# pansanity666/TransHuman

Hardware: AMD Instinct MI355X
Metric: rays/sec (512x512, 64 samples/ray) (higher is better)
Workload: dtype f32 (fp16 hi/lo x3 MFMA emulation)

## Files before the change

### transhuman_amd/csrc/k_mlp_fused8_kernel.h

```cpp
#pragma once
#include "k_mlp_fused_kernel.h"

typedef float f8_f4 __attribute__((ext_vector_type(4)));
typedef short f8_s4 __attribute__((ext_vector_type(4)));
typedef short f8_s8 __attribute__((ext_vector_type(8)));

#define F8_THREADS 512
#define F8_PART_FLOATS (3 * 8 * 32)
#define F8_PSTR 12
#define F8_MISC_FLOATS (F8_PSTR * 32 + F8_PART_FLOATS + 32 + 8)
#define F8_LDS_BYTES (ABUF_BYTES + MBUF_BYTES + F8_MISC_FLOATS * 4)
static_assert(F8_LDS_BYTES <= 163840, "the 8-wave tile must fit the CU's LDS");

#define F8_MFMA(A, B, C) __builtin_amdgcn_mfma_f32_16x16x32_f16((A), (B), (C), 0, 0, 0)

template <int CT>
__device__ __forceinline__ void f8_load_w(const uint4* __restrict__ wl, int t, uint4 (&w)[CT][2]) {
    const uint4* p = wl + (long long)t * (CT * 2 * 64);
#pragma unroll
    for (int c = 0; c < CT; ++c) {
        w[c][0] = p[(c * 2 + 0) * 64];
        w[c][1] = p[(c * 2 + 1) * 64];
    }
}
// ... 115 lines not shown
__device__ __forceinline__ void f8_gemm_rt(const char* __restrict__ ahi, const char* __restrict__ alo, int str,
                                           const uint4* __restrict__ wp, int T, int lane, f8_f4 (&acc)[CT][RT], uint4 (&w)[2][CT][2]) {
    if constexpr (RT % 3 == 0) f8_gemm3<RT, CT, ROWSTEP, PERM, PRE>(ahi, alo, str, wp, T, lane, acc, w);
    else f8_gemm<RT, CT, ROWSTEP, PERM, PRE>(ahi, alo, str, wp, T, lane, acc, w);
}

template <int STR, bool NONNEG = true>
__device__ __forceinline__ void f8_store_h(const f8_f4& t, int row, int col0, char* __restrict__ hi, char* __restrict__ lo, int lane,
                                           unsigned& rm) {
    const int c = col0 + 4 * (lane >> 4);
    uint2 a, b;
    split_pair(t[0], t[1], a.x, b.x);
    split_pair(t[2], t[3], a.y, b.y);
    range_acc<NONNEG>(rm, a.x);
    range_acc<NONNEG>(rm, a.y);
    *reinterpret_cast<uint2*>(hi + row * STR + 2 * c) = a;
    *reinterpret_cast<uint2*>(lo + row * STR + 2 * c) = b;
}
__device__ __forceinline__ f8_f4 f8_finish(const f8_f4& a, const float4& b, float inv_scale, bool relu) {
    const f32x2 sc = {inv_scale, inv_scale};
    f32x2 y01 = __builtin_elementwise_fma((f32x2){a[0], a[1]}, sc, (f32x2){b.x, b.y});
    f32x2 y23 = __builtin_elementwise_fma((f32x2){a[2], a[3]}, sc, (f32x2){b.z, b.w});
    if (relu) {
        y01 = __builtin_elementwise_max(y01, (f32x2){0.f, 0.f});
        y23 = __builtin_elementwise_max(y23, (f32x2){0.f, 0.f});
    }
    return (f8_f4){y01[0], y01[1], y23[0], y23[1]};
}
__device__ __forceinline__ float f8_xor(float v, int lane, int mask) {
    return __builtin_bit_cast(float, __builtin_amdgcn_ds_bpermute((lane ^ mask) << 2, __builtin_bit_cast(int, v)));
}
__device__ __forceinline__ float4 f8_bias(const float* __restrict__ bias, int col0, int lane) {
    return *reinterpret_cast<const float4*>(bias + col0 + 4 * (lane >> 4));
}

template <int RT, int NV, int H, int R0, bool FIRST>
__device__ __forceinline__ void f8_mfma_dual(const uint4 (&r3)[2][2], const uint4 (&ra)[1][2], const h8 (&mh)[1], const h8 (&ml)[1],
                                             const h8 (&xh)[NV], const h8 (&xl)[NV], f8_f4 (&a3)[2][2], f8_f4 (&va)[1][RT]) {
    const f8_f4 zero = {0.f, 0.f, 0.f, 0.f};
#pragma unroll
    for (int t = 0; t < 3; ++t) {
        const int wp = t == 0 ? 1 : 0;
        const bool lo = t == 1;
        const bool first = FIRST && t == 0;
        a3[0][H] = F8_MFMA(*reinterpret_cast<const h8*>(&r3[0][wp]), lo ? ml[0] : mh[0], first ? zero : a3[0][H]);
#pragma unroll
        for (int r = 0; r < NV; ++r) {
            va[0][R0 + r] = F8_MFMA(*reinterpret_cast<const h8*>(&ra[0][wp]), lo ? xl[r] : xh[r], first ? zero : va[0][R0 + r]);
            if (r == 0) a3[1][H] = F8_MFMA(*reinterpret_cast<const h8*>(&r3[1][wp]), lo ? ml[0] : mh[0], first ? zero : a3[1][H]);
        }
    }
}

template <int V>
__global__ __launch_bounds__(F8_THREADS, 2) void mlp_fused8_kernel(FusedParams P_arg) {
#define PK P_arg
    struct F8Dbg { long long* dbg; };
    const F8Dbg P{PK.dbg};
    extern __shared__ __attribute__((aligned(16))) char lds[];
    char* abuf = lds;
    char* mbuf = lds + ABUF_BYTES;
    float* misc = reinterpret_cast<float*>(lds + ABUF_BYTES + MBUF_BYTES);
    float* probs = misc;
    float* part = misc + F8_PSTR * 32;
    float* sig = part + F8_PART_FLOATS;
    int* flag = reinterpret_cast<int*>(sig + 32);

    const int tid = threadIdx.x, lane = tid & 63, wave = tid >> 6;
    const int l15 = lane & 15, g4 = lane >> 4;
    const int tile = (int)((blockIdx.x & 7) * (gridDim.x >> 3) + (blockIdx.x >> 3));
    const int pbase = tile * FM_PTS;
    if (pbase >= PK.P) return;
    const int npts = min(FM_PTS, PK.P - pbase);
    const int fm_dbg_tile = tile;
    const int zoff = 0;
    constexpr int ROWS = 32 * V, RT = 2 * V;
    constexpr int RS256 = 16 * STR256;
    int dbg_i = 1;
    long long dbg_t = 0;
    long long* dbg_keep = reinterpret_cast<long long*>(flag + 2);
    constexpr float inv_v = 1.0f / (float)V;
    unsigned rmax = 0u;
    unsigned seen_s = 0u, seen_p = 0u, seen_n = 0u, seen_i = 0u, seen_4 = 0u;
    char* a256_lo = abuf + ROWS * STR256;

    struct TexPre { unsigned h0, h1; fm_u4 rq; };
    auto tex_fetch = [&]() __attribute__((always_inline)) {
        int tl = tile;
        asm volatile("" : "+s"(tl));
        TexPre t;
        const unsigned* hb = PK.tex_hdr + (long long)tl * 512;
        t.h0 = hb[lane];
        t.h1 = hb[64 + lane];
        t.rq = (fm_u4){0u, 0u, 0u, 0u};
        if (tid < 64 * V) t.rq = *reinterpret_cast<const fm_u4*>(PK.tex_rec + (long long)tl * V * 32 * 8 + tid * 4);
        return t;
    };
    auto fill_tex = [&](const TexPre& pre, auto rgb, auto&& under) __attribute__((always_inline)) {
        constexpr bool RGB = decltype(rgb)::value;
        constexpr int TSTR = 1040, TMAX = 103, NK = (TMAX + 7) / 8, NR = 4 * V;
        static_assert(TMAX * TSTR <= ABUF_BYTES, "a pass of texel rows must fit the operand buffer");
        int wv = __builtin_amdgcn_readfirstlane(wave), tl = tile;
        asm volatile("" : "+s"(wv), "+s"(tl));
        const unsigned* hb = PK.tex_hdr + (long long)tl * 512;
        unsigned h0 = pre.h0, h1 = pre.h1;
        const int npass = __builtin_amdgcn_readfirstlane((int)(h0 >> 16));
        char* recl = reinterpret_cast<char*>(misc);
        static_assert(32 * V * 32 <= (F8_PSTR * 32 + F8_PART_FLOATS) * 4, "row records must fit probs + part");
        unsigned fv[NR][4] = {};
        f32x2 bias_lo = {0.f, 0.f}, bias_hi = {0.f, 0.f};
        if constexpr (!RGB) {
            const float4 b4 = *reinterpret_cast<const float4*>(PK.ar0.bias + 4 * lane);
            bias_lo = (f32x2){b4.x, b4.y};
            bias_hi = (f32x2){b4.z, b4.w};
        }
        for (int p = 0; p < npass; ++p) {
            if (p > 0) {
                FM_SYNCL();
                h0 = hb[p * 128 + lane];
                h1 = hb[p * 128 + 64 + lane];
            }
            const int U = __builtin_amdgcn_readfirstlane((int)(h0 & 0xffffu));
            {
                constexpr int NA = 7, NB = 10;
                const char* mbase = reinterpret_cast<const char*>(RGB ? PK.tex_map2 : PK.tex_map);
                const unsigned loff = (unsigned)lane * 16u;
                const int last = U - 1;
                fm_u4 ta[NA], tb[NB - NA], tc[NK - NB];
#pragma unroll
                for (int k = 0; k < NA; ++k) {
                    const int i = min(wv + 8 * k, last);
                    const unsigned id = (unsigned)__builtin_amdgcn_readlane((int)h0, 8 + i);
                    ta[k] = *reinterpret_cast<const fm_u4*>(mbase + TX_ADDR(id));
                }
                const bool more = U > 8 * NA, most = U > 8 * NB;
                if (more) {
#pragma unroll
                    for (int k = NA; k < NB; ++k) {
                        const int i = min(wv + 8 * k, last);
                        const unsigned id = (unsigned)__builtin_amdgcn_readlane((int)h1, i - 56);
                        tb[k - NA] = *reinterpret_cast<const fm_u4*>(mbase + TX_ADDR(id));
                    }
                }
                if (most) {
#pragma unroll
                    for (int k = NB; k < NK; ++k) {
                        const int i = min(wv + 8 * k, last);
                        const unsigned id = (unsigned)__builtin_amdgcn_readlane((int)h1, i - 56);
                        tc[k - NB] = *reinterpret_cast<const fm_u4*>(mbase + TX_ADDR(id));
                    }
                }
                if (p == 0) {
                    under();
                    if (tid < 64 * V) *reinterpret_cast<fm_u4*>(recl + tid * 16) = pre.rq;
                }
                int wv2 = wv;
                asm volatile("" : "+s"(wv2));
#pragma unroll
                for (int k = 0; k < NA; ++k) *reinterpret_cast<fm_u4*>(abuf + min(wv2 + 8 * k, last) * TSTR + lane * 16) = ta[k];
                if (more) {
#pragma unroll
                    for (int k = NA; k < NB; ++k) *reinterpret_cast<fm_u4*>(abuf + min(wv2 + 8 * k, last) * TSTR + lane * 16) = tb[k - NA];
                }
                if (most) {
#pragma unroll
                    for (int k = NB; k < NK; ++k) *reinterpret_cast<fm_u4*>(abuf + min(wv2 + 8 * k, last) * TSTR + lane * 16) = tc[k - NB];
                }
            }
            FM_SYNCL();
            const int sh2 = npass == 1 ? 2 : npass == 2 ? 1 : 0;
            const int cofs = lane * 16;
            struct RowIn { float4 a, b, c, d; fm_u4 q0; };
            auto issue = [&](int k, const fm_u4& o, RowIn& r) __attribute__((always_inline)) {
                r.q0 = *reinterpret_cast<const fm_u4*>(recl + (wv + 8 * k) * 32);
                r.a = *reinterpret_cast<const float4*>(abuf + (o[0] + cofs));
                r.b = *reinterpret_cast<const float4*>(abuf + (o[1] + cofs));
                r.c = *reinterpret_cast<const float4*>(abuf + (o[2] + cofs));
                r.d = *reinterpret_cast<const float4*>(abuf + (o[3] + cofs));
            };
            auto offs = [&](int k) __attribute__((always_inline)) {
                return *reinterpret_cast<const fm_u4*>(recl + (wv + 8 * k) * 32 + 16);
            };
            auto blend = [&](int k, const RowIn& r, auto sel) __attribute__((always_inline)) {
                const unsigned u0 = r.q0[0], u1 = r.q0[1], u2 = r.q0[2], u3 = r.q0[3];
                const float w00 = __builtin_bit_cast(float, u0), w01 = __builtin_bit_cast(float, u1),
                            w10 = __builtin_bit_cast(float, u2), w11 = __builtin_bit_cast(float, u3);
                const f32x2 W00 = {w00, w00}, W01 = {w01, w01}, W10 = {w10, w10}, W11 = {w11, w11};
                f32x2 lo = (f32x2){r.a.x, r.a.y} * W00, hi = (f32x2){r.a.z, r.a.w} * W00;
                lo = __builtin_elementwise_fma((f32x2){r.b.x, r.b.y}, W01, lo);
                hi = __builtin_elementwise_fma((f32x2){r.b.z, r.b.w}, W01, hi);
                lo = __builtin_elementwise_fma((f32x2){r.c.x, r.c.y}, W10, lo);
                hi = __builtin_elementwise_fma((f32x2){r.c.z, r.c.w}, W10, hi);
                lo = __builtin_elementwise_fma((f32x2){r.d.x, r.d.y}, W11, lo);
                hi = __builtin_elementwise_fma((f32x2){r.d.z, r.d.w}, W11, hi);
                unsigned n0, n1, n2, n3;
                if constexpr (RGB) {
                    const float l0 = lo[0], l1 = lo[1], h0f = hi[0], h1f = hi[1];
                    n0 = __builtin_bit_cast(unsigned, l0); n1 = __builtin_bit_cast(unsigned, l1);
                    n2 = __builtin_bit_cast(unsigned, h0f); n3 = __builtin_bit_cast(unsigned, h1f);
                } else {
                    lo = __builtin_elementwise_max(lo + bias_lo, (f32x2){0.f, 0.f});
                    hi = __builtin_elementwise_max(hi + bias_hi, (f32x2){0.f, 0.f});
                    split_pair(lo[0], lo[1], n0, n2);
                    split_pair(hi[0], hi[1], n1, n3);
                }
                if constexpr (decltype(sel)::value) {
                    const bool mine = ((k & 3) >> sh2) == p;
                    fv[k][0] = mine ? n0 : fv[k][0]; fv[k][1] = mine ? n1 : fv[k][1];
                    fv[k][2] = mine ? n2 : fv[k][2]; fv[k][3] = mine ? n3 : fv[k][3];
                } else {
                    fv[k][0] = n0; fv[k][1] = n1; fv[k][2] = n2; fv[k][3] = n3;
                }
            };
            auto rows_loop = [&](auto sel) __attribute__((always_inline)) {
                RowIn in[2];
                fm_u4 of[2];
                of[0] = offs(0);
                of[1] = offs(1);
                issue(0, of[0], in[0]);
#pragma unroll
                for (int k = 0; k < NR; ++k) {
                    if (k + 1 < NR) issue(k + 1, of[(k + 1) & 1], in[(k + 1) & 1]);
                    if (k + 2 < NR) of[k & 1] = offs(k + 2);
                    FM_SB();
                    blend(k, in[k & 1], sel);
                    FM_SB();
                }
            };
            if (npass == 1) rows_loop(std::false_type{});
            else rows_loop(std::true_type{});
        }
        FM_SYNCL();
        if constexpr (RGB) {
#pragma unroll
            for (int k = 0; k < NR; ++k)
                *reinterpret_cast<fm_u4*>(abuf + (wv + 8 * k) * TSTR + lane * 16) = (fm_u4){fv[k][0], fv[k][1], fv[k][2], fv[k][3]};
        } else {
#pragma unroll
            for (int k = 0; k < NR; ++k) {
                range_acc<true>(rmax, fv[k][0]);
                range_acc<true>(rmax, fv[k][1]);
                *reinterpret_cast<uint2*>(abuf + (wv + 8 * k) * STR256 + lane * 8) = make_uint2(fv[k][0], fv[k][1]);
                *reinterpret_cast<uint2*>(a256_lo + (wv + 8 * k) * STR256 + lane * 8) = make_uint2(fv[k][2], fv[k][3]);
            }
            range_commit(PK.range, TH_RANGE_P, seen_p, rmax);
        }
    };

    if (PK.dbg != nullptr && tid == 0 && (tile & 15) == 0) {
        atomicAdd(reinterpret_cast<unsigned long long*>(PK.dbg), 1ull);
        dbg_t = clock64();
        dbg_keep[0] = dbg_t;
        dbg_keep[1] = wall_clock64();
    }
    fm_u4 rv4 = {0u, 0u, 0u, 0u};
    unsigned rv1 = 0u;
    static_assert(TH_RANGE_S == 1 && TH_RANGE_P == 2 && TH_RANGE_N == 3 && TH_RANGE_INTER == 4 && TH_RANGE_F4 == 5, "range slots 1..5");
    if (PK.range != nullptr) {
        const unsigned* rtab = PK.range + zoff;
        rv4 = (fm_u4){rtab[1], rtab[2], rtab[3], rtab[4]};
        rv1 = rtab[5];
    }
    TexPre tex_pre = tex_fetch(), tex_pre2;

    int vsel[2] = {0, 0};
    float vdv[2] = {0.f, 0.f};
    f8_f4 acc2[2][RT];
    {
        constexpr int STOK_STR = 1040;
        static_assert(32 * V * STOK_STR <= ABUF_BYTES, "T' rows must fit the operand buffer");
        char* pe_hi = mbuf;
        char* pe_lo = mbuf + 32 * STR64;
        const int pt = tid & 255, prow = pt >> 3, pc = pt & 7, ppl = tid >> 8;
        const int psrc = min(prow, npts - 1);
        const uint4 pe_v = *reinterpret_cast<const uint4*>(PK.pe + (long long)(pbase + psrc) * 128 + 64 * ppl + 8 * pc);
        char* wsp_hi = mbuf + 16384;
        char* wsp_lo = wsp_hi + 32 * STRVD;
        const unsigned* hdr = reinterpret_cast<const unsigned*>(PK.stok) + (long long)((PK.P + 31) / 32 * 32) * 16 + (long long)tile * 128;
        const unsigned h0 = hdr[lane], h1 = hdr[64 + lane];
        const int ns = tid / 7, nk = tid - 7 * ns;
        int slot = -1;
        float nw = 0.f;
        if (tid < 224) {
// ... 240 lines not shown
                    f8_store_h<STR256>(n, (2 * i + h) * 16 + l15, wave * 32 + c * 16, abuf, a256_lo, lane, rmax);
                }
            }
        }
        range_commit(PK.range, TH_RANGE_N, seen_n, rmax);
    }

    uint4 wk2[2][2][2];
    FM_SB();
    f8_load_w<2>(F8_WSLICE(PK.w16.fc_2, wave, 2) + lane, 0, wk2[0]);
#pragma unroll
    for (int q = 0; q < 2; ++q) {
        const int i = tid + F8_THREADS * q, row = i >> 5, c = i & 31;
        int x = pbase + row;
        if (PK.vd_sel != nullptr && PK.rgb_all != 2 && c < 27 && row < npts) x = PK.vd_sel[pbase + row];
        vsel[q] = x;
    }
    FM_SYNCL();
    f8_gemm_rt<RT, 2, RS256, true, true>(abuf, a256_lo, STR256, F8_WSLICE(PK.w16.fc_2, wave, 2), 8, lane, acc2, wk2);
    const float4 bi[2] = {f8_bias(PK.fc_2.bias, wave * 32, lane), f8_bias(PK.fc_2.bias, wave * 32 + 16, lane)};
#pragma unroll
    for (int q = 0; q < 2; ++q) {
        const int i = tid + F8_THREADS * q, row = i >> 5, c = i & 31;
        float x = 0.f;
        if (PK.rgb_all != 2 && c < 27 && row < npts) {
            const long long vr = PK.vd_sel ? (long long)(vsel[q] / PK.vd_div) : (long long)(pbase + row);
            x = PK.vd[vr * 27 + c];
        }
        vdv[q] = x;
    }
    FM_SYNCL();
#pragma unroll
    for (int c = 0; c < 2; ++c) {
#pragma unroll
        for (int r = 0; r < RT; ++r) acc2[c][r] = f8_finish(acc2[c][r], bi[c], PK.fc_2.inv_scale, true);
#pragma unroll
        for (int h = 0; h < 2; ++h) {
            f8_f4 m = acc2[c][h];
#pragma unroll
            for (int r = 1; r < V; ++r) m = m + acc2[c][2 * r + h];
            m = m * (f8_f4){inv_v, inv_v, inv_v, inv_v};
            f8_store_h<STR256>(m, h * 16 + l15, wave * 32 + c * 16, mbuf, mbuf + 32 * STR256, lane, rmax);
        }
#pragma unroll
        for (int r = 0; r < RT; ++r) f8_store_h<STR256>(acc2[c][r], r * 16 + l15, wave * 32 + c * 16, abuf, a256_lo, lane, rmax);
    }
    range_commit(PK.range, TH_RANGE_INTER, seen_i, rmax);
    FM_SYNCL();

    char* vd_hi = mbuf + MBUF_VD_OFF;
    char* vd_lo = vd_hi + 32 * STRVD;
    tex_pre2 = tex_fetch();
    f8_f4 va[1][RT];
    {
        f8_f4 a3[2][2];
        const float4 aw[2] = {f8_bias(PK.alpha_w, wave * 32, lane), f8_bias(PK.alpha_w, wave * 32 + 16, lane)};
        const float4 b3[2] = {f8_bias(PK.fc_3.bias, wave * 32, lane), f8_bias(PK.fc_3.bias, wave * 32 + 16, lane)};
        if (PK.rgb_all != 2) {
            constexpr int T = 8;
            const uint4* w3l = F8_WSLICE(PK.w16.fc_3, wave, 2) + lane;
            const uint4* wal = F8_WSLICE(PK.w16.vfA, wave, 1) + lane;
            const int aoff = f8_aoff<true>(lane, STR256);
            const char* mhi = mbuf;
            const char* mlo = mbuf + 32 * STR256;
            uint4 r3[2][2][2], ra[2][1][2];
            h8 mah[1], mal[1], xah[V], xal[V], mbh[1], mbl[1], xbh[V], xbl[V];
            f8_load_w<2>(w3l, 0, r3[0]);
            f8_load_w<1>(wal, 0, ra[0]);
            f8_load_x<1, RS256, true>(mhi, mlo, aoff, 0, mah, mal);
            f8_load_x<V, RS256, true>(abuf, a256_lo, aoff, 0, xah, xal);
            FM_SB();
            auto step = [&](auto first, auto par, int t) __attribute__((always_inline)) {
                constexpr bool F = decltype(first)::value;
                constexpr int PB = decltype(par)::value;
                const int tn = t + 1 < T ? t + 1 : T - 1;
                f8_load_x<1, RS256, true>(mhi + RS256, mlo + RS256, aoff, t, mbh, mbl);
                f8_load_x<V, RS256, true>(abuf + V * RS256, a256_lo + V * RS256, aoff, t, xbh, xbl);
                f8_load_w<2>(w3l, tn, r3[PB ^ 1]);
                f8_load_w<1>(wal, tn, ra[PB ^ 1]);
                f8_mfma_dual<RT, V, 0, 0, F>(r3[PB], ra[PB], mah, mal, xah, xal, a3, va);
                f8_interleave<2 + 2 * V + 6, 3 * (2 + V)>();
                f8_load_x<1, RS256, true>(mhi, mlo, aoff, tn, mah, mal);
                f8_load_x<V, RS256, true>(abuf, a256_lo, aoff, tn, xah, xal);
                f8_mfma_dual<RT, V, 1, V, F>(r3[PB], ra[PB], mbh, mbl, xbh, xbl, a3, va);
                f8_interleave<2 + 2 * V, 3 * (2 + V)>();
            };
            step(std::true_type{}, std::integral_constant<int, 0>{}, 0);
            step(std::false_type{}, std::integral_constant<int, 1>{}, 1);
#pragma unroll 1
            for (int t = 2; t < T; t += 2) {
                step(std::false_type{}, std::integral_constant<int, 0>{}, t);
                step(std::false_type{}, std::integral_constant<int, 1>{}, t + 1);
            }
        } else {
#pragma unroll
            for (int r = 0; r < RT; ++r) va[0][r] = (f8_f4){0.f, 0.f, 0.f, 0.f};
            uint4 w3[2][2][2];
            f8_gemm<2, 2, RS256, true, false>(mbuf, mbuf + 32 * STR256, STR256, F8_WSLICE(PK.w16.fc_3, wave, 2), 8, lane, a3, w3);
        }
        float s2[2];
#pragma unroll
        for (int h = 0; h < 2; ++h) {
            float s = 0.f;
#pragma unroll
            for (int c = 0; c < 2; ++c) {
                const f8_f4 y = f8_finish(a3[c][h], b3[c], PK.fc_3.inv_scale, true);
                s = fmaf(y[0], aw[c].x, s);
                s = fmaf(y[1], aw[c].y, s);
                s = fmaf(y[2], aw[c].z, s);
                s = fmaf(y[3], aw[c].w, s);
            }
            s += f8_xor(s, lane, 16);
            s += f8_xor(s, lane, 32);
            s2[h] = s;
        }
        if (g4 == 0) part[wave * 32 + l15] = s2[0];
        if (g4 == 1) part[wave * 32 + 16 + l15] = s2[1];
        if (tid == 0) *flag = 0;
        FM_SYNCL();
        if (tid < 32) {
            float sg = PK.alpha_b[zoff];
#pragma unroll
            for (int w = 0; w < 8; ++w) sg += part[w * 32 + tid];
            sig[tid] = sg;
            if (tid < npts && PK.rgb_all != 2 && (PK.rgb_all == 1 || sg > 0.f)) *flag = 1;
        }
#pragma unroll
        for (int q = 0; q < 2; ++q) {
            const int i = tid + F8_THREADS * q, row = i >> 5, c = i & 31;
            _Float16 a, b;
            split_h(vdv[q], a, b);
            *reinterpret_cast<_Float16*>(vd_hi + row * STRVD + 2 * c) = a;
            *reinterpret_cast<_Float16*>(vd_lo + row * STRVD + 2 * c) = b;
        }
        FM_SYNCL();
    }
    const bool need_rgb = *flag != 0;
    float rgb_out[3] = {0.f, 0.f, 0.f};
    if (need_rgb) {
        uint4 wvd[1][2];
        f8_load_w<1>(F8_WSLICE(PK.w16.vfD, wave, 1) + lane, 0, wvd);
        FM_SB();
        fill_tex(tex_pre2, std::true_type{}, [&]() __attribute__((always_inline)) {
            h8 xh[2], xl[2];
            f8_load_x<2, 16 * STRVD, false>(vd_hi, vd_lo, f8_aoff<false>(lane, STRVD), 0, xh, xl);
#pragma unroll
            for (int r = 0; r < RT; ++r) {
                va[0][r] = F8_MFMA(*reinterpret_cast<const h8*>(&wvd[0][1]), xh[r & 1], va[0][r]);
                va[0][r] = F8_MFMA(*reinterpret_cast<const h8*>(&wvd[0][0]), xl[r & 1], va[0][r]);
                va[0][r] = F8_MFMA(*reinterpret_cast<const h8*>(&wvd[0][0]), xh[r & 1], va[0][r]);
            }
        });
        FM_SYNCL();
        uint4 w4[4][1][2];
        {
            const uint4* wl4 = F8_WSLICE(PK.w16.fc_4, wave, 1) + lane;
#pragma unroll
            for (int t = 0; t < 4; ++t) f8_load_w<1>(wl4, t, w4[t]);
        }
        float4 rw[3];
#pragma unroll
        for (int o = 0; o < 3; ++o) rw[o] = f8_bias(PK.rgb_w + o * 128, wave * 16, lane);
        const float4 b4 = f8_bias(PK.fc_4.bias, wave * 16, lane);
        const float4 bt = f8_bias(PK.rst.bias, wave * 16, lane), br = f8_bias(PK.rst.bias, 128 + wave * 16, lane);
        char* f4_hi = mbuf + MBUF_FC4_OFF;
        char* f4_lo = f4_hi + 32 * STR128;
        {
            const char* mb = abuf + l15 * 1040 + 4 * (wave * 16 + 4 * g4);
            f8_f4 u[RT];
#pragma unroll
            for (int r = 0; r < RT; ++r) {
                const float4 m1 = *reinterpret_cast<const float4*>(mb + r * 16 * 1040);
                const float4 m2 = *reinterpret_cast<const float4*>(mb + r * 16 * 1040 + 512);
                const f8_f4 t = f8_finish(va[0][r], bt, PK.rst.inv_scale, false);
                const f32x2 z2 = {0.f, 0.f};
                const f32x2 u01 = __builtin_elementwise_max((f32x2){t[0], t[1]} + (f32x2){m1.x, m1.y}, z2) + ((f32x2){m2.x, m2.y} + (f32x2){br.x, br.y});
                const f32x2 u23 = __builtin_elementwise_max((f32x2){t[2], t[3]} + (f32x2){m1.z, m1.w}, z2) + ((f32x2){m2.z, m2.w} + (f32x2){br.z, br.w});
                u[r] = (f8_f4){u01[0], u01[1], u23[0], u23[1]};
            }
#pragma unroll
            for (int h = 0; h < 2; ++h) {
                f8_f4 m = u[h];
#pragma unroll
                for (int r = 1; r < V; ++r) m = m + u[2 * r + h];
                m = m * (f8_f4){inv_v, inv_v, inv_v, inv_v};
                f8_store_h<STR128, false>(m, h * 16 + l15, wave * 16, f4_hi, f4_lo, lane, rmax);
            }
            range_commit(PK.range, TH_RANGE_F4, seen_4, rmax);
        }
        FM_SYNCL();
        f8_f4 a4[1][2];
        {
            const int aoff4 = f8_aoff<false>(lane, STR128);
#pragma unroll
// ... 48 lines not shown
```

### transhuman_amd/csrc/k_mlp_fused_host.hip

```cpp
#include <stdio.h>
#include <stdlib.h>
#include <string.h>

#include "k_mlp_fused_kernel.h"
#include "k_mlp_fused8_kernel.h"

__global__ void pack_fused_kernel(const float* __restrict__ W, int N, int K, int KB, int CT, const int* __restrict__ cols,
                                  float scale, uint4* __restrict__ out) {
    long long total = 4LL * KB * CT * 2 * 64;
    for (long long o = blockIdx.x * (long long)blockDim.x + threadIdx.x; o < total;
         o += (long long)gridDim.x * blockDim.x) {
        int lane = (int)(o & 63);
        long long q = o >> 6;
        int plane = (int)(q & 1); q >>= 1;
        int ct = (int)(q % CT); q /= CT;
        int kb = (int)(q % KB);
        int wave = (int)(q / KB);
        int col = cols[wave * CT + ct] + (lane & 31);
        int k0 = 16 * kb + 8 * (lane >> 5);
        h8 v;
#pragma unroll
        for (int j = 0; j < 8; ++j) {
            int k = k0 + j;
            float x = (col < N && k < K) ? W[(long long)col * K + k] * scale : 0.f;
// ... 310 lines not shown
    hipLaunchKernelGGL(absmax_kernel, dim3(64), dim3(256), 0, s, tprime, (long long)rows * 256, amax);
    hipLaunchKernelGGL(tok_split_kernel, dim3(th_cdiv(rows, 4) < 1024 ? th_cdiv(rows, 4) : 1024), dim3(256), 0, s, tprime, rows, sc,
                       range);
    TH_LAUNCH_CHECK();
    return 0;
}

int th_map_fold_launch(const FusedParams& base, const float* map_split, int V, int H, int W, const int32_t* box, float* fold,
                       unsigned int* range, hipStream_t s, const unsigned* demand) {
    TH_REQUIRE(base.compact_ready, "the map fold needs the colour-folded layers (th_mlp_weights.upsample_color)");
    TH_REQUIRE(V >= 1 && H >= 1 && W >= 1 && map_split && fold, "bad argument");
    MapFoldParams p;
    p.ar0 = base.ar0c; p.rst = base.rstc;
    p.lat = map_split; p.rgb = map_split + (size_t)V * H * W * 256;
    p.box = box; p.V = V; p.H = H; p.W = W;
    p.out0 = fold; p.out12 = fold + (size_t)V * H * W * 256;
    p.range = range;
    p.list = nullptr; p.count = nullptr;
    static unsigned long long attr_done = 0ull;
    if (th_lds_attr_needed(&attr_done)) {
        TH_HIP(hipFuncSetAttribute((const void*)map_fold_kernel<false>, hipFuncAttributeMaxDynamicSharedMemorySize, 2 * MF_TEX * STR272));
        TH_HIP(hipFuncSetAttribute((const void*)map_fold_kernel<true>, hipFuncAttributeMaxDynamicSharedMemorySize, 2 * MF_TEX * STR272));
    }
    if (demand != nullptr) {
        const size_t NW = (size_t)V * H * W / 32;
        p.count = demand + 2 * NW;
        p.list = reinterpret_cast<const int32_t*>(demand + 2 * NW + 16);
        hipLaunchKernelGGL(map_fold_kernel<true>, dim3(512), dim3(256), 2 * MF_TEX * STR272, s, p);
        TH_LAUNCH_CHECK();
        return 0;
    }
    const int tpr = (W + MF_TEX - 1) / MF_TEX;
    hipLaunchKernelGGL(map_fold_kernel<false>, dim3((unsigned)(V * H * tpr)), dim3(256), 2 * MF_TEX * STR272, s, p);
    TH_LAUNCH_CHECK();
    return 0;
}

int th_mlp_fused_forward(const FusedParams& base, const ThMlpPacked& heads, int V, int P, const float* stok,
                         const void* pe, const void* f, int f_ld, const float* vd, const int32_t* vd_sel, int vd_div, int rgb_all, float* raw_c,
                         unsigned int* range, hipStream_t s, const void* tsplit, const float* t_inv, int t_nc, const float* tex_map,
                         size_t tex_stride) {
    if (P <= 0) return 0;
    TH_REQUIRE(V >= 1 && V <= 3, "fused MLP supports 1..3 reference views");
    TH_REQUIRE(f_ld == 384 || (f_ld == 272 && base.compact_ready),
               "pixel-feature rows must be 384 wide, or 272 wide with upsample_color weights uploaded");
    const bool cf = f_ld == 272;
    FusedParams p = base;
    if (cf) { p.ar0 = base.ar0c; p.rst = base.rstc; }
    p.alpha_w = heads.alpha_w; p.alpha_b = heads.alpha_b; p.rgb_w = heads.rgb_w; p.rgb_b = heads.rgb_b;
    TH_REQUIRE(tsplit == nullptr || (t_inv != nullptr && t_nc >= 7 && t_nc <= 4096), "split token table: scale word and 7 <= N_c <= 4096");
    p.tsplit = (const _Float16*)tsplit; p.t_inv = t_inv; p.t_nc = t_nc;
    const bool tex = tex_map != nullptr;
    TH_REQUIRE(!tex || (cf && f != nullptr), "texel hand-over: compact (272-wide) operand planes only");
    p.tex_hdr = nullptr; p.tex_rec = nullptr; p.tex_map = nullptr; p.tex_map2 = nullptr;
    if (tex) {
        p.tex_hdr = (const unsigned*)f;
        p.tex_rec = p.tex_hdr + (size_t)th_cdiv(P, FM_PTS) * 512;
        p.tex_map = tex_map;
        p.tex_map2 = tex_map + tex_stride;
        f = nullptr;
    }
    p.stok = stok; p.pe = (const _Float16*)pe; p.f = (const _Float16*)f; p.vd = vd; p.vd_sel = vd_sel; p.vd_div = vd_div > 0 ? vd_div : 1; p.raw_c = raw_c; p.P = P; p.rgb_all = rgb_all; p.range = range;
    static unsigned long long attr_done = 0ull;
    if (th_lds_attr_needed(&attr_done)) {
#define FM_ATTR(V_, F_)                                                                                       \
    TH_HIP(hipFuncSetAttribute((const void*)mlp_fused_kernel<V_, F_>, hipFuncAttributeMaxDynamicSharedMemorySize, \
                               FUSED_LDS_BYTES))
        FM_ATTR(1, 0); FM_ATTR(2, 0); FM_ATTR(3, 0); FM_ATTR(1, 1); FM_ATTR(2, 1); FM_ATTR(3, 1);
#undef FM_ATTR
#define FM_ATTR_T(V_)                                                                                              \
    TH_HIP(hipFuncSetAttribute((const void*)mlp_fused_kernel<V_, 1, true>, hipFuncAttributeMaxDynamicSharedMemorySize, \
                               FUSED_LDS_BYTES))
        FM_ATTR_T(1); FM_ATTR_T(2); FM_ATTR_T(3);
#undef FM_ATTR_T
    }
    dim3 grid(tex ? 8 * th_cdiv(th_cdiv(P, FM_PTS), 8) : th_cdiv(P, FM_PTS));
    const bool eight = base.waves == 8 && tex && tsplit != nullptr;
    static unsigned long long attr8_done = 0ull;
    if (eight && th_lds_attr_needed(&attr8_done)) {
        TH_HIP(hipFuncSetAttribute((const void*)mlp_fused8_kernel<1>, hipFuncAttributeMaxDynamicSharedMemorySize, F8_LDS_BYTES));
        TH_HIP(hipFuncSetAttribute((const void*)mlp_fused8_kernel<2>, hipFuncAttributeMaxDynamicSharedMemorySize, F8_LDS_BYTES));
        TH_HIP(hipFuncSetAttribute((const void*)mlp_fused8_kernel<3>, hipFuncAttributeMaxDynamicSharedMemorySize, F8_LDS_BYTES));
    }
    static int dbg_state = getenv("TH_FUSED_DBG") ? 1 : 0;
    static long long* dbg_dev = nullptr;
    p.dbg = base.cycles_buf;
    const bool dbg_now = dbg_state == 1 && P >= 4096 && base.cycles_buf == nullptr;
    hipEvent_t dbg_e0 = nullptr, dbg_e1 = nullptr;
    if (dbg_now) {
        if (!dbg_dev) TH_HIP(hipMalloc((void**)&dbg_dev, 64 * sizeof(long long)));
        TH_HIP(hipMemsetAsync(dbg_dev, 0, 64 * sizeof(long long), s));
        p.dbg = dbg_dev;
        TH_HIP(hipEventCreate(&dbg_e0));
        TH_HIP(hipEventCreate(&dbg_e1));
        TH_HIP(hipStreamSynchronize(s));
        TH_HIP(hipEventRecord(dbg_e0, s));
    }
#define FM_LAUNCH(V_, F_) hipLaunchKernelGGL((mlp_fused_kernel<V_, F_>), grid, dim3(256), FUSED_LDS_BYTES, s, p)
#define FM_LAUNCH_T(V_) hipLaunchKernelGGL((mlp_fused_kernel<V_, 1, true>), grid, dim3(256), FUSED_LDS_BYTES, s, p)
#define FM_LAUNCH_8(V_) hipLaunchKernelGGL((mlp_fused8_kernel<V_>), grid, dim3(F8_THREADS), F8_LDS_BYTES, s, p)
    if (eight) {
        if (V == 1) FM_LAUNCH_8(1); else if (V == 2) FM_LAUNCH_8(2); else FM_LAUNCH_8(3);
    } else if (tex) {
        if (V == 1) FM_LAUNCH_T(1); else if (V == 2) FM_LAUNCH_T(2); else FM_LAUNCH_T(3);
    } else
    switch (V * 2 + (cf ? 1 : 0)) {
        case 2: FM_LAUNCH(1, 0); break;
        case 3: FM_LAUNCH(1, 1); break;
// ... 33 lines not shown
```

### transhuman_amd/csrc/th_internal.h

```cpp
#pragma once
#include <hip/hip_runtime.h>
#include <stdint.h>
#include <stddef.h>
#include <time.h>
#include <string>

#include "transhuman_hip.h"

#define TH_WAVE 64

void th_set_error(const std::string& msg);
#define TH_FAIL(msg)                                                                \
    do {                                                                            \
        th_set_error(std::string(__func__) + ": " + (msg));                         \
        return -1;                                                                  \
    } while (0)
#define TH_REQUIRE(cond, msg)                                                       \
    do {                                                                            \
        if (!(cond)) TH_FAIL(msg);                                                  \
    } while (0)
#define TH_HIP(call)                                                                \
    do {                                                                            \
        hipError_t e__ = (call);                                                    \
        if (e__ != hipSuccess) {                                                    \
// ... 157 lines not shown
}

#endif

struct ThMlpPacked {
    ThPacked fc_0, alpha_res_0, kv0, kv1, fc_1, fc_2, fc_3, feature_fc, rgb_res_0, view_fc, rgb_res_1, fc_4;
    ThPacked fc_0tok;
    ThPacked alpha_res_0c, rgb_res_0c, rgb_res_1c;
    bool compact_ready = false;
    float *alpha_w = nullptr, *alpha_b = nullptr;
    float *rgb_w = nullptr, *rgb_b = nullptr;
    bool ready = false;
};
struct ThVitBlockPacked {
    float *ln1_w, *ln1_b, *ln2_w, *ln2_b;
    ThPacked qkv, proj, fc1, fc2;
};
struct ThVitPacked {
    int depth = 0, dim = 0, heads = 0;
    ThVitBlockPacked* blocks = nullptr;
    float *norm_w = nullptr, *norm_b = nullptr;
    bool ready = false;
};

struct FusedLayer {
    const uint4* w;
    const float* bias;
    float inv_scale;
    int CT, KB;
    float inv_scale2;
};
struct Fused16 {
    FusedLayer fc_0pe, kv1, kv0, fc_2, fc_3, fc_4, vfA, vfD;
};
struct FusedParams {
    Fused16 w16;
    int waves;
    FusedLayer fc_0pe;
    FusedLayer kv1, ar0, kv0, fc_1, fc_2, fc_3, fc_4;
    FusedLayer vfA, vfD, rst;
    FusedLayer ar0c, rstc;
    bool compact_ready;
    const float *alpha_w, *alpha_b, *rgb_w, *rgb_b;
    const float* stok;
    const _Float16* tsplit;
    const float* t_inv;
    int t_nc;
    const _Float16* pe;
    const _Float16* f;
    const unsigned* tex_hdr;
    const unsigned* tex_rec;
    const float* tex_map;
    const float* tex_map2;
    const float* vd;
    const int32_t* vd_sel;
    int vd_div;
    float* raw_c;
    int P;
    int rgb_all;
    unsigned int* range;
    long long* dbg;
    long long* cycles_buf;
};
enum { TH_RANGE_F = 0, TH_RANGE_S = 1, TH_RANGE_P = 2, TH_RANGE_N = 3, TH_RANGE_INTER = 4, TH_RANGE_F4 = 5, TH_RANGE_CONV = 6,
       TH_RANGE_VIT = 7 };
size_t th_fused_pack_bytes();
int th_fused_pack(const th_mlp_weights* w, const th_linear* folded, void* store, FusedParams* out, hipStream_t s);
int th_mlp_fused_forward(const FusedParams& base, const ThMlpPacked& heads, int V, int P, const float* stok,
                         const void* pe, const void* f, int f_ld, const float* vd, const int32_t* vd_sel, int vd_div, int rgb_all,
                         float* raw_c, unsigned int* range, hipStream_t s, const void* tsplit = nullptr,
                         const float* t_inv = nullptr, int t_nc = 0, const float* tex_map = nullptr, size_t tex_stride = 0);
static inline bool th_lds_attr_needed(unsigned long long* done) {
    int dev = 0;
    if (hipGetDevice(&dev) != hipSuccess || dev < 0 || dev > 63) return true;
    if ((*done >> dev) & 1ull) return false;
    *done |= 1ull << dev;
    return true;
}
int th_map_fold_launch(const FusedParams& base, const float* map_split, int V, int H, int W, const int32_t* box, float* fold,
                       unsigned int* range, hipStream_t s, const unsigned* demand = nullptr );
size_t th_pixtex_bytes(int V, long long P);
int th_pixtex_launch(int V, int H, int W, const ThPointSrc* ps, const int32_t* sel, int P, const float* cams,
                     const float* scale, void* out, hipStream_t s);
int th_tok_split(float* tprime, int rows, float* sc, unsigned int* range, hipStream_t s);

struct th_ctx {
    void* fused_store = nullptr;
    FusedParams fused{};
    bool fused_ready = false;
    int mlp_mode = 1;
    int vit_mode = 1;
    int tok_gather = 1;
    int tex_rows = 1;
    int device = 0;
    void* mlp_store = nullptr;
    void* vit_store = nullptr;
    ThMlpPacked mlp;
    ThVitPacked vit;
    int32_t* host_pinned = nullptr;
    struct Prepass {
        hipEvent_t ev = nullptr;
        const void* ws = nullptr;
        const void* rays = nullptr;
        int R = 0, S = 0;
        bool valid = false;
        hipEvent_t ev2 = nullptr;
// ... 172 lines not shown
```

Before: 18.85 million.

## Stream texel rows straight to LDS with global_load_lds and partial waits

Texel row gathers no longer go through VGPRs and then LDS stores. Each wave now issues global_load_lds_dwordx4 DMA requests straight into the operand buffer, with row addresses spread across lanes by ds_bpermute. The ar0 bias row is DMA'd into LDS the same way. For the single-pass V=3 case, a new tex_hw parameter counts which rows come from the first half of the map, so the kernel waits only partially (vmcnt) and adds a mid-loop barrier once the rest arrive, overlapping the blend with the tail of the fetch. The vfD weight load is also hoisted ahead of the need_rgb branch. This aims to cut VGPR pressure and store latency, at the cost of inline asm that manipulates m0 and fragile hand-counted waitcnt logic.

```diff
diff --git a/transhuman_amd/csrc/k_mlp_fused8_kernel.h b/transhuman_amd/csrc/k_mlp_fused8_kernel.h
--- a/transhuman_amd/csrc/k_mlp_fused8_kernel.h
+++ b/transhuman_amd/csrc/k_mlp_fused8_kernel.h
@@ -191,6 +191,14 @@
     }
 }
 
+__device__ __forceinline__ void f8_dma_row(const char* gbase, unsigned voff, unsigned ldst) {
+    unsigned keep;
+    asm volatile("s_mov_b32 %0, m0\n\ts_mov_b32 m0, %3\n\ts_nop 4\n\tglobal_load_lds_dwordx4 %1, %2\n\ts_mov_b32 m0, %0"
+                 : "=&s"(keep)
+                 : "v"(voff), "s"(gbase), "s"(ldst)
+                 : "memory");
+}
+
 template <int V>
 __global__ __launch_bounds__(F8_THREADS, 2) void mlp_fused8_kernel(FusedParams P_arg) {
 #define PK P_arg
@@ -245,129 +253,156 @@
         unsigned h0 = pre.h0, h1 = pre.h1;
         const int npass = __builtin_amdgcn_readfirstlane((int)(h0 >> 16));
         char* recl = reinterpret_cast<char*>(misc);
-        static_assert(32 * V * 32 <= (F8_PSTR * 32 + F8_PART_FLOATS) * 4, "row records must fit probs + part");
-        unsigned fv[NR][4] = {};
+        static_assert(32 * V * 32 + 1024 <= (F8_PSTR * 32 + F8_PART_FLOATS) * 4, "row records + the bias row must fit probs + part");
+        char* biasl = recl + 32 * V * 32;
+        unsigned fv[NR][4];
         f32x2 bias_lo = {0.f, 0.f}, bias_hi = {0.f, 0.f};
-        if constexpr (!RGB) {
-            const float4 b4 = *reinterpret_cast<const float4*>(PK.ar0.bias + 4 * lane);
-            bias_lo = (f32x2){b4.x, b4.y};
-            bias_hi = (f32x2){b4.z, b4.w};
-        }
-        for (int p = 0; p < npass; ++p) {
+        const unsigned long long mbase = (unsigned long long)reinterpret_cast<size_t>(RGB ? PK.tex_map2 : PK.tex_map);
+        const unsigned loff = (unsigned)lane * 16u;
+        const unsigned lbase = (unsigned)(size_t)(fm_lptr)abuf;
+        const int cofs = lane * 16;
+        int p = 0, sh2 = 2;
+        struct RowIn { float4 a, b, c, d; fm_u4 q0; };
+        auto issue = [&](int k, const fm_u4& o, RowIn& r) __attribute__((always_inline)) {
+            r.q0 = *reinterpret_cast<const fm_u4*>(recl + (wv + 8 * k) * 32);
+            r.a = *reinterpret_cast<const float4*>(abuf + (o[0] + cofs));
+            r.b = *reinterpret_cast<const float4*>(abuf + (o[1] + cofs));
+            r.c = *reinterpret_cast<const float4*>(abuf + (o[2] + cofs));
+            r.d = *reinterpret_cast<const float4*>(abuf + (o[3] + cofs));
+        };
+        auto offs = [&](int k) __attribute__((always_inline)) {
+            return *reinterpret_cast<const fm_u4*>(recl + (wv + 8 * k) * 32 + 16);
+        };
+        auto blend = [&](int k, const RowIn& r, auto sel) __attribute__((always_inline)) {
+            const unsigned u0 = r.q0[0], u1 = r.q0[1], u2 = r.q0[2], u3 = r.q0[3];
+            const float w00 = __builtin_bit_cast(float, u0), w01 = __builtin_bit_cast(float, u1),
+                        w10 = __builtin_bit_cast(float, u2), w11 = __builtin_bit_cast(float, u3);
+            const f32x2 W00 = {w00, w00}, W01 = {w01, w01}, W10 = {w10, w10}, W11 = {w11, w11};
+            f32x2 lo = (f32x2){r.a.x, r.a.y} * W00, hi = (f32x2){r.a.z, r.a.w} * W00;
+            lo = __builtin_elementwise_fma((f32x2){r.b.x, r.b.y}, W01, lo);
+            hi = __builtin_elementwise_fma((f32x2){r.b.z, r.b.w}, W01, hi);
+            lo = __builtin_elementwise_fma((f32x2){r.c.x, r.c.y}, W10, lo);
+            hi = __builtin_elementwise_fma((f32x2){r.c.z, r.c.w}, W10, hi);
+            lo = __builtin_elementwise_fma((f32x2){r.d.x, r.d.y}, W11, lo);
+            hi = __builtin_elementwise_fma((f32x2){r.d.z, r.d.w}, W11, hi);
+            unsigned n0, n1, n2, n3;
+            if constexpr (RGB) {
+                const float l0 = lo[0], l1 = lo[1], h0f = hi[0], h1f = hi[1];
+                n0 = __builtin_bit_cast(unsigned, l0); n1 = __builtin_bit_cast(unsigned, l1);
+                n2 = __builtin_bit_cast(unsigned, h0f); n3 = __builtin_bit_cast(unsigned, h1f);
+            } else {
+                lo = __builtin_elementwise_max(lo + bias_lo, (f32x2){0.f, 0.f});
+                hi = __builtin_elementwise_max(hi + bias_hi, (f32x2){0.f, 0.f});
+                split_pair(lo[0], lo[1], n0, n2);
+                split_pair(hi[0], hi[1], n1, n3);
+            }
+            if constexpr (decltype(sel)::value) {
+                const bool mine = ((k & 3) >> sh2) == p;
+                fv[k][0] = mine ? n0 : fv[k][0]; fv[k][1] = mine ? n1 : fv[k][1];
+                fv[k][2] = mine ? n2 : fv[k][2]; fv[k][3] = mine ? n3 : fv[k][3];
+            } else {
+                fv[k][0] = n0; fv[k][1] = n1; fv[k][2] = n2; fv[k][3] = n3;
+            }
+        };
+        auto request_rows = [&](int U) __attribute__((always_inline)) {
+            const int c = (U + 7) >> 3;
+            const int il = min(wv + 8 * lane, U - 1);
+            const unsigned ida = (unsigned)__builtin_amdgcn_ds_bpermute((il + 8) << 2, (int)h0);
+            const unsigned idb = (unsigned)__builtin_amdgcn_ds_bpermute((il - 56) << 2, (int)h1);
+            const unsigned long long ga = mbase + ((unsigned long long)(il < 56 ? ida : idb) << 10);
+            const int alo = (int)(unsigned)ga, ahi = (int)(unsigned)(ga >> 32), ald = (int)(lbase + (unsigned)il * TSTR);
+            __builtin_amdgcn_s_waitcnt(0x0F70);
+            if constexpr (!RGB) {
+                if (p == 0 && wv == 0)
+                    f8_dma_row(reinterpret_cast<const char*>(PK.ar0.bias), loff,
+                               (unsigned)__builtin_amdgcn_readfirstlane((int)(unsigned)(size_t)(fm_lptr)biasl));
+            }
+#pragma unroll
+            for (int j = 0; j < NK; ++j) {
+                if (j < c) {
+                    const unsigned lo = (unsigned)__builtin_amdgcn_readlane(alo, j), hi = (unsigned)__builtin_amdgcn_readlane(ahi, j);
+                    f8_dma_row(reinterpret_cast<const char*>(((unsigned long long)hi << 32) | lo), loff,
+                               (unsigned)__builtin_amdgcn_readlane(ald, j));
+                }
+            }
+            return c;
+        };
+        auto bias_read = [&]() __attribute__((always_inline)) {
+            if constexpr (!RGB) {
+                const float4 b4 = *reinterpret_cast<const float4*>(biasl + 16 * lane);
+                bias_lo = (f32x2){b4.x, b4.y};
+                bias_hi = (f32x2){b4.z, b4.w};
+            }
+        };
+        auto pass_single = [&](auto sel) __attribute__((always_inline)) {
             if (p > 0) {
                 FM_SYNCL();
                 h0 = hb[p * 128 + lane];
                 h1 = hb[p * 128 + 64 + lane];
             }
+            request_rows(__builtin_amdgcn_readfirstlane((int)(h0 & 0xffffu)));
+            if (p == 0) {
+                under();
+                if (tid < 64 * V) *reinterpret_cast<fm_u4*>(recl + tid * 16) = pre.rq;
+            }
+            asm volatile("s_waitcnt vmcnt(0)" ::: "memory");
+            FM_SYNCL();
+            if (p == 0) bias_read();
+            RowIn in[2];
+            fm_u4 of[2];
+            of[0] = offs(0);
+            of[1] = offs(1);
+            issue(0, of[0], in[0]);
+#pragma unroll
+            for (int k = 0; k < NR; ++k) {
+                if (k + 1 < NR) issue(k + 1, of[(k + 1) & 1], in[(k + 1) & 1]);
+                if (k + 2 < NR) of[k & 1] = offs(k + 2);
+                FM_SB();
+                blend(k, in[k & 1], sel);
+                FM_SB();
+            }
+        };
+        if (npass > 1) {
+#pragma unroll
+            for (int k = 0; k < NR; ++k) fv[k][0] = fv[k][1] = fv[k][2] = fv[k][3] = 0u;
+            sh2 = npass == 2 ? 1 : 0;
+            for (p = 0; p < npass; ++p) pass_single(std::true_type{});
+        } else if constexpr (V != 3) {
+            pass_single(std::false_type{});
+        } else {
             const int U = __builtin_amdgcn_readfirstlane((int)(h0 & 0xffffu));
-            {
-                constexpr int NA = 7, NB = 10;
-                const char* mbase = reinterpret_cast<const char*>(RGB ? PK.tex_map2 : PK.tex_map);
-                const unsigned loff = (unsigned)lane * 16u;
-                const int last = U - 1;
-                fm_u4 ta[NA], tb[NB - NA], tc[NK - NB];
-#pragma unroll
-                for (int k = 0; k < NA; ++k) {
-                    const int i = min(wv + 8 * k, last);
-                    const unsigned id = (unsigned)__builtin_amdgcn_readlane((int)h0, 8 + i);
-                    ta[k] = *reinterpret_cast<const fm_u4*>(mbase + TX_ADDR(id));
+            const unsigned hw = PK.tex_hw;
+            const int vs0 = __builtin_popcountll(__builtin_amdgcn_ballot_w64(lane >= 8 && lane - 8 < U && h0 < hw)) +
+                            __builtin_popcountll(__builtin_amdgcn_ballot_w64(lane + 56 < U && h1 < hw));
+            const int c = request_rows(U);
+            const int spare = hw != 0u ? c - ((vs0 + 7) >> 3) : 0;
+            under();
+            if (tid < 64 * V) *reinterpret_cast<fm_u4*>(recl + tid * 16) = pre.rq;
+            if (spare >= 6) asm volatile("s_waitcnt vmcnt(6)" ::: "memory");
+            else if (spare >= 4) asm volatile("s_waitcnt vmcnt(4)" ::: "memory");
+            else if (spare >= 2) asm volatile("s_waitcnt vmcnt(2)" ::: "memory");
+            else asm volatile("s_waitcnt vmcnt(0)" ::: "memory");
+            FM_SYNCL();
+            bias_read();
+            RowIn in[2];
+            fm_u4 of[2];
+            of[0] = offs(0);
+            of[1] = offs(1);
+            issue(0, of[0], in[0]);
+#pragma unroll
+            for (int k = 0; k < NR; ++k) {
+                const bool edge = k + 1 == 4;
+                if (k + 1 < NR && !edge) issue(k + 1, of[(k + 1) & 1], in[(k + 1) & 1]);
+                if (k + 2 < NR) of[k & 1] = offs(k + 2);
+                FM_SB();
+                blend(k, in[k & 1], std::false_type{});
+                FM_SB();
+                if (edge) {
+                    asm volatile("s_waitcnt vmcnt(0)" ::: "memory");
+                    FM_LDS_BARRIER();
+                    issue(k + 1, of[(k + 1) & 1], in[(k + 1) & 1]);
                 }
-                const bool more = U > 8 * NA, most = U > 8 * NB;
-                if (more) {
-#pragma unroll
-                    for (int k = NA; k < NB; ++k) {
-                        const int i = min(wv + 8 * k, last);
-                        const unsigned id = (unsigned)__builtin_amdgcn_readlane((int)h1, i - 56);
-                        tb[k - NA] = *reinterpret_cast<const fm_u4*>(mbase + TX_ADDR(id));
-                    }
-                }
-                if (most) {
-#pragma unroll
-                    for (int k = NB; k < NK; ++k) {
-                        const int i = min(wv + 8 * k, last);
-                        const unsigned id = (unsigned)__builtin_amdgcn_readlane((int)h1, i - 56);
-                        tc[k - NB] = *reinterpret_cast<const fm_u4*>(mbase + TX_ADDR(id));
-                    }
-                }
-                if (p == 0) {
-                    under();
-                    if (tid < 64 * V) *reinterpret_cast<fm_u4*>(recl + tid * 16) = pre.rq;
-                }
-                int wv2 = wv;
-                asm volatile("" : "+s"(wv2));
-#pragma unroll
-                for (int k = 0; k < NA; ++k) *reinterpret_cast<fm_u4*>(abuf + min(wv2 + 8 * k, last) * TSTR + lane * 16) = ta[k];
-                if (more) {
-#pragma unroll
-                    for (int k = NA; k < NB; ++k) *reinterpret_cast<fm_u4*>(abuf + min(wv2 + 8 * k, last) * TSTR + lane * 16) = tb[k - NA];
-                }
-                if (most) {
-#pragma unroll
-                    for (int k = NB; k < NK; ++k) *reinterpret_cast<fm_u4*>(abuf + min(wv2 + 8 * k, last) * TSTR + lane * 16) = tc[k - NB];
-                }
-            }
-            FM_SYNCL();
-            const int sh2 = npass == 1 ? 2 : npass == 2 ? 1 : 0;
-            const int cofs = lane * 16;
-            struct RowIn { float4 a, b, c, d; fm_u4 q0; };
-            auto issue = [&](int k, const fm_u4& o, RowIn& r) __attribute__((always_inline)) {
-                r.q0 = *reinterpret_cast<const fm_u4*>(recl + (wv + 8 * k) * 32);
-                r.a = *reinterpret_cast<const float4*>(abuf + (o[0] + cofs));
-                r.b = *reinterpret_cast<const float4*>(abuf + (o[1] + cofs));
-                r.c = *reinterpret_cast<const float4*>(abuf + (o[2] + cofs));
-                r.d = *reinterpret_cast<const float4*>(abuf + (o[3] + cofs));
-            };
-            auto offs = [&](int k) __attribute__((always_inline)) {
-                return *reinterpret_cast<const fm_u4*>(recl + (wv + 8 * k) * 32 + 16);
-            };
-            auto blend = [&](int k, const RowIn& r, auto sel) __attribute__((always_inline)) {
-                const unsigned u0 = r.q0[0], u1 = r.q0[1], u2 = r.q0[2], u3 = r.q0[3];
-                const float w00 = __builtin_bit_cast(float, u0), w01 = __builtin_bit_cast(float, u1),
-                            w10 = __builtin_bit_cast(float, u2), w11 = __builtin_bit_cast(float, u3);
-                const f32x2 W00 = {w00, w00}, W01 = {w01, w01}, W10 = {w10, w10}, W11 = {w11, w11};
-                f32x2 lo = (f32x2){r.a.x, r.a.y} * W00, hi = (f32x2){r.a.z, r.a.w} * W00;
-                lo = __builtin_elementwise_fma((f32x2){r.b.x, r.b.y}, W01, lo);
-                hi = __builtin_elementwise_fma((f32x2){r.b.z, r.b.w}, W01, hi);
-                lo = __builtin_elementwise_fma((f32x2){r.c.x, r.c.y}, W10, lo);
-                hi = __builtin_elementwise_fma((f32x2){r.c.z, r.c.w}, W10, hi);
-                lo = __builtin_elementwise_fma((f32x2){r.d.x, r.d.y}, W11, lo);
-                hi = __builtin_elementwise_fma((f32x2){r.d.z, r.d.w}, W11, hi);
-                unsigned n0, n1, n2, n3;
-                if constexpr (RGB) {
-                    const float l0 = lo[0], l1 = lo[1], h0f = hi[0], h1f = hi[1];
-                    n0 = __builtin_bit_cast(unsigned, l0); n1 = __builtin_bit_cast(unsigned, l1);
-                    n2 = __builtin_bit_cast(unsigned, h0f); n3 = __builtin_bit_cast(unsigned, h1f);
-                } else {
-                    lo = __builtin_elementwise_max(lo + bias_lo, (f32x2){0.f, 0.f});
-                    hi = __builtin_elementwise_max(hi + bias_hi, (f32x2){0.f, 0.f});
-                    split_pair(lo[0], lo[1], n0, n2);
-                    split_pair(hi[0], hi[1], n1, n3);
-                }
-                if constexpr (decltype(sel)::value) {
-                    const bool mine = ((k & 3) >> sh2) == p;
-                    fv[k][0] = mine ? n0 : fv[k][0]; fv[k][1] = mine ? n1 : fv[k][1];
-                    fv[k][2] = mine ? n2 : fv[k][2]; fv[k][3] = mine ? n3 : fv[k][3];
-                } else {
-                    fv[k][0] = n0; fv[k][1] = n1; fv[k][2] = n2; fv[k][3] = n3;
-                }
-            };
-            auto rows_loop = [&](auto sel) __attribute__((always_inline)) {
-                RowIn in[2];
-                fm_u4 of[2];
-                of[0] = offs(0);
-                of[1] = offs(1);
-                issue(0, of[0], in[0]);
-#pragma unroll
-                for (int k = 0; k < NR; ++k) {
-                    if (k + 1 < NR) issue(k + 1, of[(k + 1) & 1], in[(k + 1) & 1]);
-                    if (k + 2 < NR) of[k & 1] = offs(k + 2);
-                    FM_SB();
-                    blend(k, in[k & 1], sel);
-                    FM_SB();
-                }
-            };
-            if (npass == 1) rows_loop(std::false_type{});
-            else rows_loop(std::true_type{});
+            }
         }
         FM_SYNCL();
         if constexpr (RGB) {
@@ -714,6 +749,7 @@
     char* vd_lo = vd_hi + 32 * STRVD;
     tex_pre2 = tex_fetch();
     f8_f4 va[1][RT];
+    uint4 wvd[1][2];
     {
         f8_f4 a3[2][2];
         const float4 aw[2] = {f8_bias(PK.alpha_w, wave * 32, lane), f8_bias(PK.alpha_w, wave * 32 + 16, lane)};
@@ -778,6 +814,7 @@
         }
         if (g4 == 0) part[wave * 32 + l15] = s2[0];
         if (g4 == 1) part[wave * 32 + 16 + l15] = s2[1];
+        f8_load_w<1>(F8_WSLICE(PK.w16.vfD, wave, 1) + lane, 0, wvd);
         if (tid == 0) *flag = 0;
         FM_SYNCL();
         if (tid < 32) {
@@ -800,8 +837,6 @@
     const bool need_rgb = *flag != 0;
     float rgb_out[3] = {0.f, 0.f, 0.f};
     if (need_rgb) {
-        uint4 wvd[1][2];
-        f8_load_w<1>(F8_WSLICE(PK.w16.vfD, wave, 1) + lane, 0, wvd);
         FM_SB();
         fill_tex(tex_pre2, std::true_type{}, [&]() __attribute__((always_inline)) {
             h8 xh[2], xl[2];
diff --git a/transhuman_amd/csrc/k_mlp_fused_host.hip b/transhuman_amd/csrc/k_mlp_fused_host.hip
--- a/transhuman_amd/csrc/k_mlp_fused_host.hip
+++ b/transhuman_amd/csrc/k_mlp_fused_host.hip
@@ -386,8 +386,9 @@
     p.tsplit = (const _Float16*)tsplit; p.t_inv = t_inv; p.t_nc = t_nc;
     const bool tex = tex_map != nullptr;
     TH_REQUIRE(!tex || (cf && f != nullptr), "texel hand-over: compact (272-wide) operand planes only");
-    p.tex_hdr = nullptr; p.tex_rec = nullptr; p.tex_map = nullptr; p.tex_map2 = nullptr;
+    p.tex_hdr = nullptr; p.tex_rec = nullptr; p.tex_map = nullptr; p.tex_map2 = nullptr; p.tex_hw = 0u;
     if (tex) {
+        p.tex_hw = (unsigned)(tex_stride / ((size_t)256 * V));
         p.tex_hdr = (const unsigned*)f;
         p.tex_rec = p.tex_hdr + (size_t)th_cdiv(P, FM_PTS) * 512;
         p.tex_map = tex_map;
diff --git a/transhuman_amd/csrc/th_internal.h b/transhuman_amd/csrc/th_internal.h
--- a/transhuman_amd/csrc/th_internal.h
+++ b/transhuman_amd/csrc/th_internal.h
@@ -233,6 +233,7 @@
     const unsigned* tex_rec;
     const float* tex_map;
     const float* tex_map2;
+    unsigned tex_hw;
     const float* vd;
     const int32_t* vd_sel;
     int vd_div;
```

Result: faster. 19.12 million (median of 6 runs) (+1.4%).
